# DredderGun/accbpg_and_fw

Hardware: AMD Instinct MI355X
Metric: D-opt iters/sec (m=2048,n=32768) (higher is better)
Workload: dtype f64; 1 GPU; D_opt_design(2048,32768) abpg_gain gamma=2 fp64, one independent instance per GPU; instances=1, instances_per_gpu=1, seeds=1..1, window=transient: iterations 5..161 from x0 = 1/n, linear_gram=False

## Files before the change

accbpg_and_fw_amd/csrc/dopt_kernels.hip:

```cpp
#include <atomic>
#include <mutex>
#include <unordered_map>
#include <type_traits>

#include "internal.h"
#include "mfma_tile.hpp"

namespace accbpg {

struct GramSeg {
    int64_t row0, col0, kb, ke;
    bool dual, whole;
};
constexpr int GRAM_RMAX = 4;
template <class T>
__device__ __forceinline__ GramSeg gram_segment(const TileRC* __restrict__ tiles, int64_t kiters, int64_t it,
                                                int64_t it1) {
    const int e = (int)(it / kiters);
    const int64_t off = it - (int64_t)e * kiters;
    const TileRC tr = tiles[e];
    GramSeg g;
    if (tr.d1 < 0) {
        g.row0 = (int64_t)tr.rb * T::BM; g.col0 = (int64_t)tr.cb * T::BN;
        g.kb = off; g.ke = min(kiters, off + (it1 - it));
// ... 1000 lines not shown
        const int c = 2 * (tid & 31), r0 = tid >> 5;
#pragma unroll
        for (int p = 0; p < 8; ++p) {
            const int r = r0 + 8 * p;
            v[p] = load2_guard(G + (int64_t)r * ld + c, r < mr, c, mc, vec_ok);
        }
    }
    __device__ __forceinline__ void to_lds(double* __restrict__ img, int st) const {
        const int tid = threadIdx.x;
        const int c = 2 * (tid & 31), r0 = tid >> 5;
#pragma unroll
        for (int p = 0; p < 8; ++p) {
            img[(r0 + 8 * p) * st + c] = v[p].x;
            img[(r0 + 8 * p) * st + c + 1] = v[p].y;
        }
    }
    __device__ __forceinline__ void from_lds(const double* __restrict__ img, int st) {
        const int tid = threadIdx.x;
        const int c = 2 * (tid & 31), r0 = tid >> 5;
#pragma unroll
        for (int p = 0; p < 8; ++p) {
            v[p].x = img[(r0 + 8 * p) * st + c];
            v[p].y = img[(r0 + 8 * p) * st + c + 1];
        }
    }
    __device__ __forceinline__ void store(double* __restrict__ G, int64_t ld, int mr, int mc, bool lower) const {
        const int tid = threadIdx.x;
        const int c = 2 * (tid & 31), r0 = tid >> 5;
#pragma unroll
        for (int p = 0; p < 8; ++p) {
            const int r = r0 + 8 * p;
            if (r < mr) {
                if (c < mc && (!lower || c <= r)) G[(int64_t)r * ld + c] = v[p].x;
                if (c + 1 < mc && (!lower || c + 1 <= r)) G[(int64_t)r * ld + c + 1] = v[p].y;
            }
        }
    }
};

__device__ __forceinline__ double rsqrt_newton(double d) {
    double y = __builtin_amdgcn_rsq(d);
    const double h = -0.5 * d;
    y = y * fma(h * y, y, 1.5);
    y = y * fma(h * y, y, 1.5);
    return y;
}

template <int SRC>
__device__ __forceinline__ double quad_bcast(double v) {
    constexpr int ctrl = SRC | (SRC << 2) | (SRC << 4) | (SRC << 6);
    int lo = __double2loint(v), hi = __double2hiint(v);
    lo = __builtin_amdgcn_mov_dpp(lo, ctrl, 0xF, 0xF, true);
    hi = __builtin_amdgcn_mov_dpp(hi, ctrl, 0xF, 0xF, true);
    return __hiloint2double(hi, lo);
}

__device__ __forceinline__ void solve16_quad(const double* P, double* X, int row, int k0,
                                             const double* __restrict__ lt, const double* __restrict__ rv) {
    const int q = threadIdx.x & 3;
    const double* prow = P + row * SP + k0;
    double* xr = X + row * SP + k0;
    double pr[4], xs[4];
#pragma unroll
    for (int t = 0; t < 4; ++t) pr[t] = prow[4 * t + q];
    double lv[2][4][4], rvv[2][4];
    auto group = [&](auto gtag) {
        constexpr int g = decltype(gtag)::value;
#pragma unroll
        for (int cc = 0; cc < 4; ++cc) {
            const int c = 4 * g + cc;
            rvv[g & 1][cc] = rv[c];
#pragma unroll
            for (int t = 0; t < 4; ++t)
                if (4 * t + 3 > c) lv[g & 1][cc][t] = lt[c * 16 + 4 * t + q];
        }
    };
    auto column = [&](auto ctag) {
        constexpr int c = decltype(ctag)::value;
        constexpr int qc = c & 3, tc = c >> 2, g = c >> 2;
        const double x = quad_bcast<qc>(pr[tc] * rvv[g & 1][c & 3]);
        xs[tc] = (q == qc) ? x : xs[tc];
#pragma unroll
        for (int t = 0; t < 4; ++t)
            if (4 * t + 3 > c) pr[t] = fma(-x, lv[g & 1][c & 3][t], pr[t]);
    };
    group(std::integral_constant<int, 0>{});
    group(std::integral_constant<int, 1>{});
    column(std::integral_constant<int, 0>{});  column(std::integral_constant<int, 1>{});
    column(std::integral_constant<int, 2>{});  column(std::integral_constant<int, 3>{});
    group(std::integral_constant<int, 2>{});
    column(std::integral_constant<int, 4>{});  column(std::integral_constant<int, 5>{});
    column(std::integral_constant<int, 6>{});  column(std::integral_constant<int, 7>{});
    group(std::integral_constant<int, 3>{});
    column(std::integral_constant<int, 8>{});  column(std::integral_constant<int, 9>{});
    column(std::integral_constant<int, 10>{}); column(std::integral_constant<int, 11>{});
    column(std::integral_constant<int, 12>{}); column(std::integral_constant<int, 13>{});
    column(std::integral_constant<int, 14>{}); column(std::integral_constant<int, 15>{});
#pragma unroll
    for (int t = 0; t < 4; ++t) xr[4 * t + q] = xs[t];
}

template <int SRC>
__device__ __forceinline__ double row_bcast(double v) {
    return __builtin_amdgcn_update_dpp(0.0, v, 0x150 + SRC, 0xF, 0xF, true);
}
#ifndef ACCBPG_DPP_ASM
#define ACCBPG_DPP_ASM 1
#endif
template <int C, int NOPS_BEFORE, int NOPS_AFTER>
__device__ __forceinline__ void fmac_row_bcast(double& acc, double l, double nl) {
#if ACCBPG_DPP_ASM
    if constexpr (NOPS_BEFORE) asm volatile("s_nop 1");
    asm volatile("v_fmac_f64_dpp %0, %1, %2 row_newbcast:%3 row_mask:0xf bank_mask:0xf"
                 : "+v"(acc)
                 : "v"(l), "v"(nl), "n"(C));
    if constexpr (NOPS_AFTER) asm volatile("s_nop 1");
#else
    acc = fma(row_bcast<C>(l), nl, acc);
#endif
}
template <int C>
__device__ __forceinline__ double mul_row_bcast(double y, double v) {
#if ACCBPG_DPP_ASM
    double out = 0.0;
    asm volatile("s_nop 1\n\tv_fmac_f64_dpp %0, %1, %2 row_newbcast:%3 row_mask:0xf bank_mask:0xf"
                 : "+v"(out)
                 : "v"(y), "v"(v), "n"(C));
    return out;
#else
    return fma(row_bcast<C>(y), v, 0.0);
#endif
}
template <int C0, int C1>
__device__ __forceinline__ void potrf16_updates(double (&a)[16], double l, double nl) {
    if constexpr (C0 < C1 && C0 < 16) {
        fmac_row_bcast<C0, 0, (C0 == 15)>(a[C0], l, nl);
        potrf16_updates<C0 + 1, C1>(a, l, nl);
    }
}
template <int J>
__device__ __forceinline__ void potrf16_step(double (&a)[16], double& l, int r, int k0, int bs, double& dsv,
                                             double& myrs, double& minp) {
    a[J] = l;
    if constexpr (J + 1 < 16) {
        const double nl = -l;
        fmac_row_bcast<J + 1, 1, 0>(a[J + 1], l, nl);
        const double p = a[J + 1];
        constexpr int N = 14 - J, Q = (N + 3) / 4;
        double y = __builtin_amdgcn_rsq(p);
        const double h = -0.5 * p;
        __builtin_amdgcn_sched_barrier(0);
        potrf16_updates<J + 2, J + 2 + Q>(a, l, nl);
        __builtin_amdgcn_sched_barrier(0);
        const double t = h * y;
        __builtin_amdgcn_sched_barrier(0);
        potrf16_updates<J + 2 + Q, J + 2 + 2 * Q>(a, l, nl);
        __builtin_amdgcn_sched_barrier(0);
        const double u = fma(t, y, 1.5);
        __builtin_amdgcn_sched_barrier(0);
        potrf16_updates<J + 2 + 2 * Q, J + 2 + 3 * Q>(a, l, nl);
        __builtin_amdgcn_sched_barrier(0);
        y = y * u;
        __builtin_amdgcn_sched_barrier(0);
        potrf16_updates<J + 2 + 3 * Q, 16>(a, l, nl);
        __builtin_amdgcn_sched_barrier(0);
        const bool mine = (r == J + 1);
        dsv = mine ? p : dsv;
        myrs = mine ? y : myrs;
        minp = (mine && (k0 + J + 1 < bs)) ? p : minp;
        l = mul_row_bcast<J + 1>(y, p);
    }
}
constexpr int POTRF_TB = 16 * 16 + 16;
struct PotrfNoHook { __device__ __forceinline__ void operator()(int, int) const {} };
template <class Hook = PotrfNoHook>
__device__ __forceinline__ void potrf64_blk(double* __restrict__ S, double* __restrict__ Lo,
                                            double* __restrict__ tbuf, int* __restrict__ badflag, int bs,
                                            int dbg = 0, Hook hook = Hook()) {
    const int tid = threadIdx.x;
    const int lane = tid & 63, wave = __builtin_amdgcn_readfirstlane(tid >> 6);
    for (int e = tid; e < 6 * 256; e += NTHREADS) {
        const int b = e >> 8, w = e & 255;
        const int br = (b < 3) ? 0 : ((b < 5) ? 1 : 2);
        const int bc = (b < 3) ? b + 1 : ((b < 5) ? b - 1 : 3);
        Lo[(16 * br + (w >> 4)) * SP + 16 * bc + (w & 15)] = 0.0;
    }
#pragma unroll 1
    for (int pnl = 0; pnl < NB / 16; ++pnl) {
        const int k0 = 16 * pnl;
        double* lt = tbuf + pnl * POTRF_TB;
        double* rv = lt + 256;
        if (wave == 0 && !(dbg & 32)) {
            const int r = lane & 15;
            double a[16];
#pragma unroll
            for (int c = 0; c < 16; ++c) a[c] = S[(k0 + r) * SP + k0 + c];
            double dsv = 1.0, myrs = 1.0, minp = 1.0;
            double l;
            {
                const double piv = row_bcast<0>(a[0]);
                const double rs = rsqrt_newton(piv);
                dsv = (r == 0) ? piv : dsv;
                myrs = (r == 0) ? rs : myrs;
                minp = (r == 0 && k0 < bs) ? piv : 1.0;
                l = a[0] * rs;
            }
            potrf16_step<0>(a, l, r, k0, bs, dsv, myrs, minp);
            potrf16_step<1>(a, l, r, k0, bs, dsv, myrs, minp);
            potrf16_step<2>(a, l, r, k0, bs, dsv, myrs, minp);
            potrf16_step<3>(a, l, r, k0, bs, dsv, myrs, minp);
            potrf16_step<4>(a, l, r, k0, bs, dsv, myrs, minp);
            potrf16_step<5>(a, l, r, k0, bs, dsv, myrs, minp);
            potrf16_step<6>(a, l, r, k0, bs, dsv, myrs, minp);
            potrf16_step<7>(a, l, r, k0, bs, dsv, myrs, minp);
            potrf16_step<8>(a, l, r, k0, bs, dsv, myrs, minp);
            potrf16_step<9>(a, l, r, k0, bs, dsv, myrs, minp);
            potrf16_step<10>(a, l, r, k0, bs, dsv, myrs, minp);
            potrf16_step<11>(a, l, r, k0, bs, dsv, myrs, minp);
            potrf16_step<12>(a, l, r, k0, bs, dsv, myrs, minp);
            potrf16_step<13>(a, l, r, k0, bs, dsv, myrs, minp);
            potrf16_step<14>(a, l, r, k0, bs, dsv, myrs, minp);
            potrf16_step<15>(a, l, r, k0, bs, dsv, myrs, minp);
            const bool bad = __any(!(minp > 0.0));
            const double dg = sqrt(dsv);
            if (lane < 16) {
#pragma unroll
                for (int c = 0; c < 16; ++c) {
                    const double v = (c < r) ? a[c] : ((c == r) ? dg : 0.0);
                    Lo[(k0 + r) * SP + k0 + c] = v;
                    lt[c * 16 + r] = v;
                }
                rv[r] = myrs;
                if (bad) *badflag = 1;
            }
        } else {
            hook(pnl, 3);
        }
        hook(pnl, 0);
        __syncthreads();
        hook(pnl, 1);
        if (pnl == NB / 16 - 1) break;
        const int nrows = NB - k0 - 16;
        if (tid < 4 * nrows && !(dbg & 8)) {
            const int row = k0 + 16 + (tid >> 2);
            solve16_quad(S, Lo, row, k0, lt, rv);
        }
        __syncthreads();
        {
            const int nb = NB / 16 - 1 - pnl;
            const int nblk = nb * (nb + 1) / 2;
            const int lr = lane & 15, lq = lane >> 4;
            for (int b = wave; b < nblk && !(dbg & 16); b += NTHREADS / 64) {
                int bi = 0;
                while ((bi + 1) * (bi + 2) / 2 <= b) ++bi;
                const int bj = b - bi * (bi + 1) / 2;
                const int ri = 16 * (pnl + 1 + bi), rj = 16 * (pnl + 1 + bj);
                d4 acc = d4{0.0, 0.0, 0.0, 0.0};
#pragma unroll
                for (int kk = 0; kk < 4; ++kk) {
                    const double av = Lo[(ri + lr) * SP + k0 + 4 * kk + lq];
                    const double bv = Lo[(rj + lr) * SP + k0 + 4 * kk + lq];
                    acc = __builtin_amdgcn_mfma_f64_16x16x4f64(av, bv, acc, 0, 0, 0);
                }
#pragma unroll
                for (int rr = 0; rr < 4; ++rr) S[(ri + lq + 4 * rr) * SP + rj + lr] -= acc[rr];
            }
        }
        __syncthreads();
    }
}

__device__ __forceinline__ void trsm64_blk(double* __restrict__ Xs, const double* __restrict__ Lo,
                                           const double* __restrict__ tbuf) {
    const int tid = threadIdx.x;
    const int lane = tid & 63, wave = __builtin_amdgcn_readfirstlane(tid >> 6);
#pragma unroll 1
    for (int pnl = 0; pnl < NB / 16; ++pnl) {
        const int k0 = 16 * pnl;
        const double* lt = tbuf + pnl * POTRF_TB;
        const double* rv = lt + 256;
        solve16_quad(Xs, Xs, tid >> 2, k0, lt, rv);
        if (pnl == NB / 16 - 1) break;
        __syncthreads();
        {
            const int ncb = NB / 16 - 1 - pnl;
            const int lr = lane & 15, lq = lane >> 4;
            for (int b = wave; b < 4 * ncb; b += NTHREADS / 64) {
                const int bi = b & 3, q = pnl + 1 + (b >> 2);
                d4 acc = d4{0.0, 0.0, 0.0, 0.0};
#pragma unroll
                for (int kk = 0; kk < 4; ++kk) {
                    const double av = Xs[(16 * bi + lr) * SP + k0 + 4 * kk + lq];
                    const double bv = Lo[(16 * q + lr) * SP + k0 + 4 * kk + lq];
                    acc = __builtin_amdgcn_mfma_f64_16x16x4f64(av, bv, acc, 0, 0, 0);
                }
#pragma unroll
                for (int rr = 0; rr < 4; ++rr) Xs[(16 * bi + lq + 4 * rr) * SP + 16 * q + lr] -= acc[rr];
            }
        }
        __syncthreads();
    }
}

template <class Fetch, class Done>
__device__ __forceinline__ bool trsm64_stream(double* __restrict__ Xs, const double* __restrict__ Lo,
                                              const double* __restrict__ tbuf, Fetch fetch, Done done) {
    const int tid = threadIdx.x;
    const int lane = tid & 63, wave = __builtin_amdgcn_readfirstlane(tid >> 6);
#pragma unroll 1
    for (int pnl = 0; pnl < NB / 16; ++pnl) {
        const int k0 = 16 * pnl;
        const double* lt = tbuf + pnl * POTRF_TB;
        const double* rv = lt + 256;
        if (!fetch(pnl, 0)) return false;
        if (pnl + 1 < NB / 16) fetch(pnl + 1, 1);
        solve16_quad(Xs, Xs, tid >> 2, k0, lt, rv);
        if (pnl + 1 < NB / 16) fetch(pnl + 1, 2);
        __syncthreads();
        if (!done(pnl)) return false;
        if (pnl == NB / 16 - 1) break;
        {
            const int ncb = NB / 16 - 1 - pnl;
            const int lr = lane & 15, lq = lane >> 4;
            for (int b = wave; b < 4 * ncb; b += NTHREADS / 64) {
                const int bi = b & 3, q = pnl + 1 + (b >> 2);
                d4 acc = d4{0.0, 0.0, 0.0, 0.0};
#pragma unroll
                for (int kk = 0; kk < 4; ++kk) {
                    const double av = Xs[(16 * bi + lr) * SP + k0 + 4 * kk + lq];
                    const double bv = Lo[(16 * q + lr) * SP + k0 + 4 * kk + lq];
                    acc = __builtin_amdgcn_mfma_f64_16x16x4f64(av, bv, acc, 0, 0, 0);
                }
#pragma unroll
                for (int rr = 0; rr < 4; ++rr) Xs[(16 * bi + lq + 4 * rr) * SP + 16 * q + lr] -= acc[rr];
            }
        }
    }
    return true;
}

__global__ __launch_bounds__(NTHREADS, 1) void chol_step_kernel(double* __restrict__ A, int64_t lda, int64_t m,
                                                               int kc, int pend, int jmax, int T,
                                                               double* __restrict__ logdet,
                                                               int* __restrict__ flags, int dbg,
                                                               double* __restrict__ Winv, double* __restrict__ Ldiag) {
    extern __shared__ __attribute__((aligned(16))) double lds[];
    double* Ak = lds;
    double* Bk = Ak + NB * SQ;
    double* S = Bk + NB * SQ;
    double* Lo = S + NB * SP;
    double* misc = Lo + NB * SP;
    int* badflag = reinterpret_cast<int*>(misc);
    double* red = misc + 8;
    const int tid = threadIdx.x;
    const int kprev = pend ? kc - 1 : -1;
    const int npanel = T - kc;
    const bool vec_ok = ((reinterpret_cast<uintptr_t>(A) & 15) == 0) && ((lda & 1) == 0);
    const double* Lk = A + (int64_t)(kc - 1) * NB;
    acc64_t acc;

    if ((int)blockIdx.x >= npanel) {
        const int u = blockIdx.x - npanel;
        int ii, jj;
        if (jmax >= T - 1) {
            ii = (int)((sqrt(8.0 * u + 1.0) - 1.0) * 0.5);
            while ((ii + 1) * (ii + 2) / 2 <= u) ++ii;
            while (ii * (ii + 1) / 2 > u) --ii;
            jj = u - ii * (ii + 1) / 2;
        } else {
            const int J = jmax - kc;
            ii = u / J; jj = u - ii * J;
            if (jj > ii) return;
        }
        const int i = kc + 1 + ii, j = kc + 1 + jj;
        const int mi = (int)min((int64_t)NB, m - (int64_t)i * NB), mj = (int)min((int64_t)NB, m - (int64_t)j * NB);
        Blk64 bi, bj, bc;
        bi.load(Lk + (int64_t)i * NB * lda, lda, mi, NB, vec_ok);
        bj.load(Lk + (int64_t)j * NB * lda, lda, mj, NB, vec_ok);
        double* Cij = A + (int64_t)i * NB * lda + (int64_t)j * NB;
        bc.load(Cij, lda, mi, mj, vec_ok);
        bi.to_lds(Ak, SQ);
        bj.to_lds(Bk, SQ);
        bc.to_lds(S, SP);
        __syncthreads();
        mma64(acc, Ak, Bk);
        sub_acc64(S, acc, mi, mj, i == j);
        __syncthreads();
        bc.from_lds(S, SP);
        bc.store(Cij, lda, mi, mj, i == j);
        return;
    }

    const int i = kc + blockIdx.x;
    const bool diag = (i == kc);
    const int bs = (int)min((int64_t)NB, m - (int64_t)kc * NB);
    const int mi = (int)min((int64_t)NB, m - (int64_t)i * NB);
    double* Akk = A + (int64_t)kc * NB * lda + (int64_t)kc * NB;
    double* Pik = A + (int64_t)i * NB * lda + (int64_t)kc * NB;
    Blk64 bkk, bik, bd, bp;
    bd.load(Akk, lda, bs, bs, vec_ok);
    if (kprev >= 0) bkk.load(Lk + (int64_t)kc * NB * lda, lda, bs, NB, vec_ok);
    if (!diag) {
        bp.load(Pik, lda, mi, bs, vec_ok);
        if (kprev >= 0) bik.load(Lk + (int64_t)i * NB * lda, lda, mi, NB, vec_ok);
    }
    {
        const int c = 2 * (tid & 31), r0 = tid >> 5;
#pragma unroll
        for (int p = 0; p < 8; ++p) {
            const int r = r0 + 8 * p;
            const bool in = r < bs;
            S[r * SP + c] = (in && c <= r) ? bd.v[p].x : ((r == c) ? 1.0 : 0.0);
            S[r * SP + c + 1] = (in && c + 1 <= r && c + 1 < bs) ? bd.v[p].y : ((r == c + 1) ? 1.0 : 0.0);
        }
    }
    if (tid == 0) *badflag = 0;
    acc64_t pacc;
    if (kprev >= 0) {
        bkk.to_lds(Bk, SQ);
        if (!diag) bik.to_lds(Ak, SQ);
        __syncthreads();
        if (!(dbg & 4)) {
            mma64(acc, Bk, Bk);
            if (!diag) mma64(pacc, Ak, Bk);
            sub_acc64(S, acc, bs, bs, true);
        }
    }
    __syncthreads();
    if (!(dbg & 1)) potrf64_blk(S, Lo, Ak, badflag, bs, dbg);
    else { __syncthreads(); for (int e = tid; e < NB * SP; e += NTHREADS) Lo[e] = S[e]; __syncthreads(); }
    const bool bad = (*badflag != 0);
    if (diag) {
        Blk64 bl;
        bl.from_lds(Lo, SP);
        bl.store(Ldiag + (int64_t)kc * NB * lda + (int64_t)kc * NB, lda, bs, bs, true);
        double lg = (tid < bs) ? log(Lo[tid * SP + tid]) : 0.0;
        for (int off = 32; off > 0; off >>= 1) lg += __shfl_down(lg, off);
        if ((tid & 63) == 0) red[tid >> 6] = lg;
        __syncthreads();
        if (tid == 0) {
#if defined(ACCBPG_PLAIN_LOGDET) && ACCBPG_PLAIN_LOGDET
            *logdet += 2.0 * (red[0] + red[1] + red[2] + red[3]);
#else
            __hip_atomic_fetch_add(logdet, 2.0 * (red[0] + red[1] + red[2] + red[3]), __ATOMIC_RELAXED,
                                   __HIP_MEMORY_SCOPE_AGENT);
#endif
            if (bad) flags[FLAG_NOT_PD] = 1;
        }
        if (Winv != nullptr) {
            __syncthreads();
            for (int e = tid; e < NB * NB; e += NTHREADS) S[(e >> 6) * SP + (e & 63)] = ((e >> 6) == (e & 63)) ? 1.0 : 0.0;
            __syncthreads();
            trsm64_blk(S, Lo, Ak);
            __syncthreads();
            double* Wkk = Winv + (int64_t)kc * NB * lda + (int64_t)kc * NB;
            for (int e = tid; e < NB * NB; e += NTHREADS) {
                const int r = e >> 6, c = e & 63;
                if (r < bs && c < bs) Wkk[(int64_t)r * lda + c] = (c <= r) ? S[c * SP + r] : 0.0;
            }
        }
        return;
    }
    double* Xs = S;
    bp.to_lds(Xs, SP);
    __syncthreads();
    if (kprev >= 0 && !(dbg & 4)) sub_acc64(Xs, pacc, mi, bs, false);
    __syncthreads();
    if (!(dbg & 2)) trsm64_blk(Xs, Lo, Ak);
    __syncthreads();
    bp.from_lds(Xs, SP);
    bp.store(Pik, lda, mi, bs, false);
}

__device__ __forceinline__ void mma64_acc(acc64_t& acc, const double* __restrict__ As, const double* __restrict__ Bs) {
    const int lane = threadIdx.x & 63, wave = __builtin_amdgcn_readfirstlane(threadIdx.x >> 6);
    const int wm = wave >> 1, wn = wave & 1;
    const int lr = lane & 15, lq = lane >> 4;
    const double* ap = As + (16 * wm + lr) * SQ + lq;
    const double* bp = Bs + (32 * wn + lr) * SQ + lq;
#pragma unroll 4
    for (int kk = 0; kk < NB / 4; ++kk) {
        const double a0 = ap[4 * kk], a1 = ap[32 * SQ + 4 * kk];
        const double b0 = bp[4 * kk], b1 = bp[16 * SQ + 4 * kk];
        acc[0][0] = __builtin_amdgcn_mfma_f64_16x16x4f64(a0, b0, acc[0][0], 0, 0, 0);
        acc[0][1] = __builtin_amdgcn_mfma_f64_16x16x4f64(a0, b1, acc[0][1], 0, 0, 0);
        acc[1][0] = __builtin_amdgcn_mfma_f64_16x16x4f64(a1, b0, acc[1][0], 0, 0, 0);
        acc[1][1] = __builtin_amdgcn_mfma_f64_16x16x4f64(a1, b1, acc[1][1], 0, 0, 0);
    }
}

__global__ __launch_bounds__(NTHREADS, 2) void chol_syrk_kernel(double* __restrict__ A, int64_t lda, int64_t m,
                                                               int k0, int nk, int T) {
    extern __shared__ __attribute__((aligned(16))) double lds[];
    double* Ak = lds;
    double* Bk = Ak + NB * SQ;
    double* S = Ak;
    const bool vec_ok = ((reinterpret_cast<uintptr_t>(A) & 15) == 0) && ((lda & 1) == 0);
    const int u = blockIdx.x;
    int ii = (int)((sqrt(8.0 * u + 1.0) - 1.0) * 0.5);
    while ((ii + 1) * (ii + 2) / 2 <= u) ++ii;
    while (ii * (ii + 1) / 2 > u) --ii;
    const int jj = u - ii * (ii + 1) / 2;
    const int i = k0 + nk + ii, j = k0 + nk + jj;
    if (i >= T) return;
    const int mi = (int)min((int64_t)NB, m - (int64_t)i * NB), mj = (int)min((int64_t)NB, m - (int64_t)j * NB);
    double* Cij = A + (int64_t)i * NB * lda + (int64_t)j * NB;
    const double* Li = A + (int64_t)i * NB * lda + (int64_t)k0 * NB;
    const double* Lj = A + (int64_t)j * NB * lda + (int64_t)k0 * NB;
    Blk64 bi, bj, bc;
    bc.load(Cij, lda, mi, mj, vec_ok);
    bi.load(Li, lda, mi, NB, vec_ok);
    bj.load(Lj, lda, mj, NB, vec_ok);
    acc64_t acc;
#pragma unroll
    for (int a = 0; a < 2; ++a)
#pragma unroll
        for (int b = 0; b < 2; ++b) acc[a][b] = d4{0.0, 0.0, 0.0, 0.0};
#pragma unroll 1
    for (int k = 0; k < nk; ++k) {
        bi.to_lds(Ak, SQ);
        bj.to_lds(Bk, SQ);
        if (k + 1 < nk) {
            bi.load(Li + (int64_t)(k + 1) * NB, lda, mi, NB, vec_ok);
            bj.load(Lj + (int64_t)(k + 1) * NB, lda, mj, NB, vec_ok);
        }
        __syncthreads();
        mma64_acc(acc, Ak, Bk);
        __syncthreads();
    }
    bc.to_lds(S, SP);
    __syncthreads();
    sub_acc64(S, acc, mi, mj, i == j);
    __syncthreads();
    bc.from_lds(S, SP);
    bc.store(Cij, lda, mi, mj, i == j);
}

constexpr int CT_TMAX = 32;
constexpr int CT_AUX = 4 * POTRF_TB + 8;
constexpr int CT_LDS_DOUBLES = 2 * NB * SQ + 4 * POTRF_TB + 16;
constexpr int CT_LDS_BYTES = CT_LDS_DOUBLES * 8;

constexpr int CT_NSTAMP = 32;

typedef __attribute__((address_space(1))) double gdouble;
typedef __attribute__((address_space(1))) int gint;
__device__ __forceinline__ double ct_ld(const double* p) {
    return __hip_atomic_load((const gdouble*)p, __ATOMIC_RELAXED, __HIP_MEMORY_SCOPE_AGENT);
}
__device__ __forceinline__ void ct_st(double* p, double v) {
    __hip_atomic_store((gdouble*)p, v, __ATOMIC_RELAXED, __HIP_MEMORY_SCOPE_AGENT);
}
__device__ __forceinline__ int ct_ldi(const int* p) {
    return __hip_atomic_load((const gint*)p, __ATOMIC_RELAXED, __HIP_MEMORY_SCOPE_AGENT);
}
__device__ __forceinline__ void ct_sti(int* p, int v) {
    __hip_atomic_store((gint*)p, v, __ATOMIC_RELAXED, __HIP_MEMORY_SCOPE_AGENT);
}
__device__ __forceinline__ bool ct_spin(const int* flag, int* abortw, long long limit) {
    if (ct_ldi(flag) != 0) return true;
    const long long t0 = wall_clock64();
    unsigned n = 0;
    for (;;) {
        __builtin_amdgcn_s_sleep(1);
        if (ct_ldi(flag) != 0) return true;
        if ((++n & 15u) == 0u) {
            if (ct_ldi(abortw) != 0) return false;
            if (wall_clock64() - t0 > limit) {
                ct_sti(abortw, 1);
                return false;
            }
        }
    }
}
__device__ __forceinline__ bool ct_wait(const int* f0, const int* f1, int* abortw, long long limit, int* word) {
    if (threadIdx.x < 64) {
        bool ok = ct_spin(f0, abortw, limit);
        if (ok && f1 != nullptr) ok = ct_spin(f1, abortw, limit);
        if (threadIdx.x == 0) *word = ok ? 1 : 0;
    }
    __syncthreads();
    return *word != 0;
}
template <int ST, bool LOWER>
__device__ __forceinline__ void ct_fetch(double* __restrict__ img, const double* G, int64_t ld, int mr, int mc) {
    const int tid = threadIdx.x;
    const int c = 2 * (tid & 31), r0 = tid >> 5;
    double v[16];
#pragma unroll
    for (int p = 0; p < 8; ++p) {
        const int r = r0 + 8 * p;
        const bool in0 = r < mr && c < mc && (!LOWER || c <= r);
        const bool in1 = r < mr && c + 1 < mc && (!LOWER || c + 1 <= r);
        v[2 * p] = in0 ? ct_ld(G + (int64_t)r * ld + c) : 0.0;
        v[2 * p + 1] = in1 ? ct_ld(G + (int64_t)r * ld + c + 1) : 0.0;
    }
#pragma unroll
    for (int p = 0; p < 8; ++p) {
        img[(r0 + 8 * p) * ST + c] = v[2 * p];
        img[(r0 + 8 * p) * ST + c + 1] = v[2 * p + 1];
    }
}
template <bool LOWER>
__device__ __forceinline__ void ct_publish(const double* __restrict__ img, double* G, int64_t ld, int mr, int mc) {
    const int tid = threadIdx.x;
    const int c = 2 * (tid & 31), r0 = tid >> 5;
#pragma unroll
    for (int p = 0; p < 8; ++p) {
        const int r = r0 + 8 * p;
        if (r < mr) {
            if (c < mc && (!LOWER || c <= r)) ct_st(G + (int64_t)r * ld + c, img[r * SP + c]);
            if (c + 1 < mc && (!LOWER || c + 1 <= r)) ct_st(G + (int64_t)r * ld + c + 1, img[r * SP + c + 1]);
        }
    }
}
__device__ __forceinline__ void ct_signal(int* flag) {
    asm volatile("s_waitcnt vmcnt(0)" ::: "memory");
    __syncthreads();
    if (threadIdx.x == 0) ct_sti(flag, 1);
}
__device__ __forceinline__ void ct_load_acc(acc64_t& acc, const double* __restrict__ G, int64_t ld, int mr, int mc) {
    const int lane = threadIdx.x & 63, wave = __builtin_amdgcn_readfirstlane(threadIdx.x >> 6);
    const int wm = wave >> 1, wn = wave & 1;
    const int lr = lane & 15, lq = lane >> 4;
#pragma unroll
    for (int i = 0; i < 2; ++i)
#pragma unroll
        for (int j = 0; j < 2; ++j)
#pragma unroll
            for (int r = 0; r < 4; ++r) {
                const int row = 16 * (2 * i + wm) + lq + 4 * r, col = 32 * wn + 16 * j + lr;
                acc[i][j][r] = (row < mr && col < mc) ? G[(int64_t)row * ld + col] : 0.0;
            }
}
template <bool DIAG>
__device__ __forceinline__ void ct_acc_to_img(double* __restrict__ img, const acc64_t& acc, int bs) {
    const int lane = threadIdx.x & 63, wave = __builtin_amdgcn_readfirstlane(threadIdx.x >> 6);
    const int wm = wave >> 1, wn = wave & 1;
    const int lr = lane & 15, lq = lane >> 4;
#pragma unroll
    for (int i = 0; i < 2; ++i)
#pragma unroll
        for (int j = 0; j < 2; ++j)
#pragma unroll
            for (int r = 0; r < 4; ++r) {
                const int row = 16 * (2 * i + wm) + lq + 4 * r, col = 32 * wn + 16 * j + lr;
                double v = acc[i][j][r];
                if (DIAG) v = (row < bs && col < bs && col <= row) ? v : ((row == col) ? 1.0 : 0.0);
                img[row * SP + col] = v;
            }
}
template <int SA, int SB>
__device__ __forceinline__ void ct_update(acc64_t& acc, const double* __restrict__ As, const double* __restrict__ Bs) {
    const int lane = threadIdx.x & 63, wave = __builtin_amdgcn_readfirstlane(threadIdx.x >> 6);
    const int wm = wave >> 1, wn = wave & 1;
    const int lr = lane & 15, lq = lane >> 4;
    const double* ap = As + (16 * wm + lr) * SA + lq;
    const double* bp = Bs + (32 * wn + lr) * SB + lq;
    d4 p00 = d4{0.0, 0.0, 0.0, 0.0}, p01 = p00, p10 = p00, p11 = p00;
#pragma unroll 4
    for (int kk = 0; kk < NB / 4; ++kk) {
        const double a0 = ap[4 * kk], a1 = ap[32 * SA + 4 * kk];
        const double b0 = bp[4 * kk], b1 = bp[16 * SB + 4 * kk];
        p00 = __builtin_amdgcn_mfma_f64_16x16x4f64(a0, b0, p00, 0, 0, 0);
        p01 = __builtin_amdgcn_mfma_f64_16x16x4f64(a0, b1, p01, 0, 0, 0);
        p10 = __builtin_amdgcn_mfma_f64_16x16x4f64(a1, b0, p10, 0, 0, 0);
        p11 = __builtin_amdgcn_mfma_f64_16x16x4f64(a1, b1, p11, 0, 0, 0);
    }
    acc[0][0] -= p00; acc[0][1] -= p01; acc[1][0] -= p10; acc[1][1] -= p11;
}

__global__ __launch_bounds__(NTHREADS, 2) void chol_tiles_kernel(CholInst one, const CholInst* __restrict__ table,
                                                                const CholJob* __restrict__ jobs, int64_t ld, int64_t m,
                                                                int T, long long spin_limit, int stall_test, BatchAct act) {
    extern __shared__ __attribute__((aligned(16))) double lds[];
    double* R0 = lds;
    double* R1 = R0 + NB * SQ;
    double* tbuf = R1 + NB * SQ;
    int* word = reinterpret_cast<int*>(tbuf + 4 * POTRF_TB);
    int* badflag = word + 2;
    double* red = tbuf + 4 * POTRF_TB + 8;

    const CholInst ci = (table != nullptr) ? table[act.idx[blockIdx.y]] : one;
    const CholJob job = jobs[blockIdx.x];
    const int tid = threadIdx.x;
    const bool diagrole = (job.i == job.j);
    const int d = job.i;
    const bool has_off = !diagrole || d > 0;
    const int ti = job.i, tj = diagrole ? d - 1 : job.j;
    int* abortw = ci.flags + FLAG_ABORT;
    int* pflags = ci.ready + T * T;
    int* hflags = pflags + 4 * T;
    auto blk = [&](int b) { return (int)min((int64_t)NB, m - (int64_t)b * NB); };
    auto at = [&](auto* base, int bi, int bj) { return base + (int64_t)bi * NB * ld + (int64_t)bj * NB; };
    if (stall_test && blockIdx.x == 0) return;
    auto stamp = [&](int slot) {
        if (ci.trace != nullptr && diagrole && tid == 0) ci.trace[d * CT_NSTAMP + slot] = wall_clock64();
    };
    stamp(0);

    acc64_t accO, accD;
    const int mi = blk(ti);
    if (has_off) ct_load_acc(accO, at(ci.src, ti, tj), ld, mi, blk(tj));
    if (diagrole && d < 2) ct_load_acc(accD, at(ci.src, d, d), ld, blk(d), blk(d));

    double run_logdet = 0.0, run_bad = 0.0;
    if (has_off) {
        for (int k = 0; k < tj; ++k) {
            if (!ct_wait(ci.ready + ti * T + k, nullptr, abortw, spin_limit, word)) return;
            ct_fetch<SQ, false>(R0, at(ci.L, ti, k), ld, mi, NB);
            if (!ct_wait(ci.ready + tj * T + k, nullptr, abortw, spin_limit, word)) return;
            ct_fetch<SQ, false>(R1, at(ci.L, tj, k), ld, blk(tj), NB);
            __syncthreads();
            ct_update<SQ, SQ>(accO, R0, R1);
        }
        __syncthreads();
        ct_acc_to_img<false>(R0, accO, NB);
        stamp(1);
        const double* ax = ci.aux + (int64_t)tj * CT_AUX;
        const double* Ljj = at(ci.Ldiag, tj, tj);
        int* pflag = pflags + 4 * tj;
        double pc_t[2], pc_l[3], pc_s[2];
        bool have = false;
        int looked = 0;
        auto load_piece = [&](int pnl) {
            const int k0 = 16 * pnl;
#pragma unroll
            for (int q = 0; q < 2; ++q) {
                const int e = tid + q * NTHREADS;
                pc_t[q] = (e < POTRF_TB) ? ct_ld(ax + pnl * POTRF_TB + e) : 0.0;
            }
#pragma unroll
            for (int q = 0; q < 3; ++q) {
                const int e = tid + q * NTHREADS;
                pc_l[q] = (e < (NB - k0 - 16) * 16) ? ct_ld(Ljj + (int64_t)(k0 + 16 + (e >> 4)) * ld + k0 + (e & 15)) : 0.0;
            }
            if (pnl == 3) {
                pc_s[0] = ct_ld(ax + 4 * POTRF_TB);
                pc_s[1] = ct_ld(ax + 4 * POTRF_TB + 1);
            }
        };
        auto land_piece = [&](int pnl) {
            const int k0 = 16 * pnl;
#pragma unroll
            for (int q = 0; q < 2; ++q) {
                const int e = tid + q * NTHREADS;
                if (e < POTRF_TB) tbuf[pnl * POTRF_TB + e] = pc_t[q];
            }
#pragma unroll
            for (int q = 0; q < 3; ++q) {
                const int e = tid + q * NTHREADS;
                if (e < (NB - k0 - 16) * 16) R1[(k0 + 16 + (e >> 4)) * SP + k0 + (e & 15)] = pc_l[q];
            }
            if (pnl == 3) { run_logdet = pc_s[0]; run_bad = pc_s[1]; }
        };
        auto fetch = [&](int pnl, int mode) -> bool {
            if (mode == 1) { looked = ct_ldi(pflag + pnl); return true; }
            if (mode == 2) { if (looked != 0) { load_piece(pnl); have = true; } return true; }
            stamp(8 + 4 * pnl + (have ? 0 : 0));
            if (have) land_piece(pnl);
            if (__syncthreads_or(have ? 0 : 1)) {
                if (!ct_wait(pflag + pnl, nullptr, abortw, spin_limit, word)) return false;
                if (!have) { load_piece(pnl); land_piece(pnl); }
                __syncthreads();
            }
            have = false;
            stamp(9 + 4 * pnl);
            if (pnl == 0) stamp(2);
            if (pnl == 3) stamp(3);
            return true;
        };
        double* Lij = at(ci.L, ti, tj);
        const int mj = blk(tj);
        d4 p00 = d4{0.0, 0.0, 0.0, 0.0}, p01 = p00, p10 = p00, p11 = p00;
        auto done = [&](int pnl) -> bool {
            const int k0 = 16 * pnl;
            stamp(10 + 4 * pnl);
            for (int e = tid; e < NB * 16; e += NTHREADS) {
                const int r = e >> 4, c = k0 + (e & 15);
                if (r < mi && c < mj) ct_st(Lij + (int64_t)r * ld + c, R0[r * SP + c]);
            }
            if (diagrole) {
                const int lane = tid & 63, wave = __builtin_amdgcn_readfirstlane(tid >> 6);
                const int wm = wave >> 1, wn = wave & 1;
                const double* ap = R0 + (16 * wm + (lane & 15)) * SP + (lane >> 4);
                const double* bp = R0 + (32 * wn + (lane & 15)) * SP + (lane >> 4);
#pragma unroll
                for (int kk = 4 * pnl; kk < 4 * pnl + 4; ++kk) {
                    const double a0 = ap[4 * kk], a1 = ap[32 * SP + 4 * kk];
                    const double b0 = bp[4 * kk], b1 = bp[16 * SP + 4 * kk];
                    p00 = __builtin_amdgcn_mfma_f64_16x16x4f64(a0, b0, p00, 0, 0, 0);
                    p01 = __builtin_amdgcn_mfma_f64_16x16x4f64(a0, b1, p01, 0, 0, 0);
                    p10 = __builtin_amdgcn_mfma_f64_16x16x4f64(a1, b0, p10, 0, 0, 0);
                    p11 = __builtin_amdgcn_mfma_f64_16x16x4f64(a1, b1, p11, 0, 0, 0);
                }
                if (pnl == 2 && d >= 2) {
                    if (!ct_wait(hflags + d, nullptr, abortw, spin_limit, word)) return false;
                    const double* hd = ci.hand + (int64_t)d * NB * NB;
#pragma unroll
                    for (int i = 0; i < 2; ++i)
#pragma unroll
                        for (int j = 0; j < 2; ++j)
#pragma unroll
                            for (int r = 0; r < 4; ++r) accD[i][j][r] = ct_ld(hd + ((i * 2 + j) * 4 + r) * NTHREADS + tid);
                }
            }
            stamp(11 + 4 * pnl);
            if (pnl == 3) stamp(4);
            return true;
        };
        if (!trsm64_stream(R0, R1, tbuf, fetch, done)) return;
        if (!diagrole) {
            ct_signal(ci.ready + ti * T + tj);
            if (tj != 0) return;
            acc64_t accH;
            ct_load_acc(accH, at(ci.src, ti, ti), ld, mi, mi);
            for (int k = 0; k + 1 < ti; ++k) {
                if (!ct_wait(ci.ready + ti * T + k, nullptr, abortw, spin_limit, word)) return;
                ct_fetch<SQ, false>(R0, at(ci.L, ti, k), ld, mi, NB);
                __syncthreads();
                ct_update<SQ, SQ>(accH, R0, R0);
            }
            double* hd = ci.hand + (int64_t)ti * NB * NB;
#pragma unroll
            for (int i = 0; i < 2; ++i)
#pragma unroll
                for (int j = 0; j < 2; ++j)
#pragma unroll
                    for (int r = 0; r < 4; ++r) ct_st(hd + ((i * 2 + j) * 4 + r) * NTHREADS + tid, accH[i][j][r]);
            ct_signal(hflags + ti);
            return;
        }
        accD[0][0] -= p00; accD[0][1] -= p01; accD[1][0] -= p10; accD[1][1] -= p11;
    }
    const int bs = blk(d);
    ct_acc_to_img<true>(R1, accD, bs);
    if (tid == 0) *badflag = 0;
    asm volatile("s_waitcnt vmcnt(0)" ::: "memory");
    __syncthreads();
    if (has_off && tid == 0) ct_sti(ci.ready + ti * T + tj, 1);
    stamp(5);
    double* axd = ci.aux + (int64_t)d * CT_AUX;
    double* Ldd = at(ci.Ldiag, d, d);
    int* pflag_d = pflags + 4 * d;
    auto publish_piece = [&](int pnl, int first, int nthr) {
        const int k0 = 16 * pnl;
        for (int e = tid - first; e < (NB - k0) * 16; e += nthr) {
            const int r = k0 + (e >> 4), c = k0 + (e & 15);
            if (r < bs && c <= r) ct_st(Ldd + (int64_t)r * ld + c, R0[r * SP + c]);
        }
        for (int e = tid - first; e < POTRF_TB; e += nthr) ct_st(axd + pnl * POTRF_TB + e, tbuf[pnl * POTRF_TB + e]);
    };
    auto hook = [&](int pnl, int where) {
        if (where == 3 && pnl > 0) publish_piece(pnl - 1, 64, NTHREADS - 64);
        else if (where == 0 && pnl > 0) asm volatile("s_waitcnt vmcnt(0)" ::: "memory");
        else if (where == 1 && pnl > 0 && tid == 0) ct_sti(pflag_d + pnl - 1, 1);
    };
    potrf64_blk(R1, R0, tbuf, badflag, bs, 0, hook);
    stamp(6);
    double lg = (tid < bs) ? log(R0[tid * SP + tid]) : 0.0;
    for (int off = 32; off > 0; off >>= 1) lg += __shfl_down(lg, off);
    if ((tid & 63) == 0) red[tid >> 6] = lg;
    publish_piece(3, 0, NTHREADS);
    __syncthreads();
    const double logdet = run_logdet + 2.0 * (red[0] + red[1] + red[2] + red[3]);
    const double bad = (*badflag != 0 || run_bad != 0.0) ? 1.0 : 0.0;
    if (tid == 0) { ct_st(axd + 4 * POTRF_TB, logdet); ct_st(axd + 4 * POTRF_TB + 1, bad); }
    ct_signal(pflag_d + 3);
    stamp(7);
    if (d == T - 1 && tid == 0) {
        *ci.logdet = logdet;
        if (bad != 0.0) ci.flags[FLAG_NOT_PD] = 1;
    }
    if (ci.Winv != nullptr) {
        for (int e = tid; e < NB * NB; e += NTHREADS) R1[(e >> 6) * SP + (e & 63)] = ((e >> 6) == (e & 63)) ? 1.0 : 0.0;
        __syncthreads();
        trsm64_blk(R1, R0, tbuf);
        __syncthreads();
        double* Wkk = at(ci.Winv, d, d);
        for (int e = tid; e < NB * NB; e += NTHREADS) {
            const int r = e >> 6, c = e & 63;
            if (r < bs && c < bs) Wkk[(int64_t)r * ld + c] = (c <= r) ? R1[c * SP + r] : 0.0;
        }
    }
}

__global__ __launch_bounds__(64) void trtri_diag_kernel(const double* __restrict__ L, int64_t ldl,
                                                       double* __restrict__ W, int64_t ldw, int64_t m) {
    __shared__ double Ls[NB * SP];
    __shared__ double Ws[NB * SP];
    __shared__ double rinv[NB];
    const int tid = threadIdx.x;
    const int64_t k0 = (int64_t)blockIdx.x * NB;
    const int bs = (int)min((int64_t)NB, m - k0);
    const double* L11 = L + k0 * ldl + k0;
    for (int e = tid; e < NB * NB; e += 64) {
        const int r = e / NB, c = e % NB;
        Ls[r * SP + c] = (r < bs && c <= r) ? L11[(int64_t)r * ldl + c] : ((r == c) ? 1.0 : 0.0);
    }
    __syncthreads();
    rinv[tid] = 1.0 / Ls[tid * SP + tid];
    __syncthreads();
    double w[NB];
#pragma unroll
    for (int r = 0; r < NB; ++r) {
        double s = (r == tid) ? 1.0 : 0.0;
#pragma unroll
        for (int c = 0; c < r; ++c) s -= Ls[r * SP + c] * w[c];
        w[r] = (r >= tid) ? s * rinv[r] : 0.0;
    }
#pragma unroll
    for (int r = 0; r < NB; ++r) Ws[r * SP + tid] = w[r];
    __syncthreads();
    double* W11 = W + k0 * ldw + k0;
    for (int e = tid; e < NB * NB; e += 64) {
        const int r = e / NB, c = e % NB;
        if (r < bs && c < bs) W11[(int64_t)r * ldw + c] = Ws[r * SP + c];
    }
}

template <bool COPY = false>
__device__ __forceinline__ bool xcheck_bad(const double* __restrict__ x, int64_t n, double* __restrict__ keep = nullptr) {
    bool bad = false;
    const int64_t step = (int64_t)blockDim.x * 8;
    int64_t i = threadIdx.x;
    for (; i + 7 * (int64_t)blockDim.x < n; i += step) {
        double v[8];
#pragma unroll
        for (int u = 0; u < 8; ++u) v[u] = x[i + u * (int64_t)blockDim.x];
#pragma unroll
        for (int u = 0; u < 8; ++u) {
            bad |= !(v[u] >= 0.0);
            if (COPY) keep[i + u * (int64_t)blockDim.x] = v[u];
        }
    }
    for (; i < n; i += blockDim.x) {
        const double v = x[i];
        bad |= !(v >= 0.0);
        if (COPY) keep[i] = v;
    }
    return __syncthreads_or(bad ? 1 : 0) != 0;
}

__global__ __launch_bounds__(1024) void zero_scalars_kernel(double* dscal, int* dflag, const double* __restrict__ x,
                                                          int64_t n, int* __restrict__ ready, int nready,
                                                          double* __restrict__ xkeep) {
#if defined(ACCBPG_PLAIN_LOGDET) && ACCBPG_PLAIN_LOGDET
    if (threadIdx.x < 8) dscal[threadIdx.x] = 0.0;
#else
    if (threadIdx.x < 8) __hip_atomic_store(dscal + threadIdx.x, 0.0, __ATOMIC_RELAXED, __HIP_MEMORY_SCOPE_AGENT);
#endif
    if (threadIdx.x < 8) dflag[threadIdx.x] = 0;
    for (int i = threadIdx.x; i < nready; i += blockDim.x) ready[i] = 0;
    if (x == nullptr) return;
    const bool bad = xkeep ? xcheck_bad<true>(x, n, xkeep) : xcheck_bad<false>(x, n);
    if (bad && threadIdx.x == 0) dflag[FLAG_NEG_X] = 1;
}

__global__ __launch_bounds__(1024) void zero_scalars_batch_kernel(const BatchInst* __restrict__ bt, BatchAct act,
                                                                const double* __restrict__ xbase, int64_t ldx, int64_t n,
                                                                int nready) {
    const int inst = act.idx[blockIdx.x];
    const BatchInst bi = bt[inst];
    if (threadIdx.x < 8) __hip_atomic_store(bi.dscal + threadIdx.x, 0.0, __ATOMIC_RELAXED, __HIP_MEMORY_SCOPE_AGENT);
    if (threadIdx.x < 8) bi.dflag[threadIdx.x] = 0;
    for (int i = threadIdx.x; i < nready; i += blockDim.x) bi.chol_ready[i] = 0;
    if (xbase == nullptr) return;
    if (xcheck_bad(xbase + (int64_t)inst * ldx, n) && threadIdx.x == 0) bi.dflag[FLAG_NEG_X] = 1;
}

__global__ void set_op_kernel(GemmOp* slot, GemmOp op) { *slot = op; }

__global__ __launch_bounds__(NTHREADS, 1) void mfma_peak_kernel(int iters, double* sink) {
    d4 acc[8];
#pragma unroll
    for (int i = 0; i < 8; ++i) acc[i] = d4{0.0, 0.0, 0.0, 0.0};
    double a = 1.0 + threadIdx.x * 1e-3, b = 0.5 - threadIdx.x * 1e-3;
    for (int it = 0; it < iters; ++it) {
#pragma unroll
        for (int i = 0; i < 8; ++i)
            asm volatile("v_mfma_f64_16x16x4_f64 %0, %1, %2, %0" : "+v"(acc[i]) : "v"(a), "v"(b));
    }
    asm volatile("s_nop 15\n\ts_nop 15" ::: "memory");
    double s = 0.0;
#pragma unroll
    for (int i = 0; i < 8; ++i) s += acc[i][0] + acc[i][1] + acc[i][2] + acc[i][3];
    if (s == 123.456) sink[0] = s;
}

__global__ __launch_bounds__(NTHREADS, 1) void pipe_probe_kernel(int iters, int mode, double* sink) {
    d4 acc[8];
    double va[16];
#pragma unroll
    for (int i = 0; i < 8; ++i) acc[i] = d4{0.0, 0.0, 0.0, 0.0};
#pragma unroll
    for (int i = 0; i < 16; ++i) va[i] = threadIdx.x * 1e-3 + i;
    double a = 1.0 + threadIdx.x * 1e-3, b = 0.5 - threadIdx.x * 1e-3;
    for (int it = 0; it < iters; ++it) {
        if (mode & 1) {
#pragma unroll
            for (int i = 0; i < 8; ++i) asm volatile("v_mfma_f64_16x16x4_f64 %0, %1, %2, %0" : "+v"(acc[i]) : "v"(a), "v"(b));
        }
        if (mode & 2) {
#pragma unroll
            for (int r = 0; r < 8; ++r)
#pragma unroll
                for (int i = 0; i < 16; ++i) asm volatile("v_fma_f64 %0, %1, %2, %0" : "+v"(va[i]) : "v"(a), "v"(b));
        }
    }
    asm volatile("s_nop 15\n\ts_nop 15" ::: "memory");
    double s = 0.0;
#pragma unroll
    for (int i = 0; i < 8; ++i) s += acc[i][0] + acc[i][1] + acc[i][2] + acc[i][3];
#pragma unroll
    for (int i = 0; i < 16; ++i) s += va[i];
    if (s == 123.456) sink[0] = s;
}

template <class K>
static int set_lds(K kernel, int bytes) {
    ACC_HIP(hipFuncSetAttribute(reinterpret_cast<const void*>(kernel), hipFuncAttributeMaxDynamicSharedMemorySize,
                                bytes));
    return ACCBPG_OK;
}

static int ensure_lds(const void* kernel, int bytes) {
    static std::mutex mu;
    static std::unordered_map<const void*, int> limit;
    std::lock_guard<std::mutex> guard(mu);
    auto it = limit.find(kernel);
    if (it != limit.end() && it->second >= bytes) return ACCBPG_OK;
    ACC_HIP(hipFuncSetAttribute(kernel, hipFuncAttributeMaxDynamicSharedMemorySize, bytes));
    limit[kernel] = bytes;
    return ACCBPG_OK;
}
#define ACC_LAUNCH_LDS(kernel, grid, block, lds, stream, ...)                        \
    do {                                                                             \
        auto k__ = kernel;                                                           \
        ACC_TRY(ensure_lds(reinterpret_cast<const void*>(k__), (int)(lds)));         \
        k__<<<(grid), (block), (lds), (stream)>>>(__VA_ARGS__);                      \
    } while (0)

void prof_begin(accbpg_dopt* h, ProfKind k) {
    if (!h->prof_on) return;
    ProfSlot& p = h->prof[k];
    if (p.used + 2 > p.ev.size()) {
        hipEvent_t a, b;
        hipEventCreate(&a);
        hipEventCreate(&b);
        p.ev.push_back(a);
        p.ev.push_back(b);
    }
    hipEventRecord(p.ev[p.used], h->stream);
}
void prof_end(accbpg_dopt* h, ProfKind k) {
    if (!h->prof_on) return;
    ProfSlot& p = h->prof[k];
    hipEventRecord(p.ev[p.used + 1], h->stream);
    p.used += 2;
    p.launches += 1;
}

static int g_plan_flags = 0;
void set_plan_flags(int flags) { g_plan_flags = flags; }

static std::atomic<int> g_gemm_loop{0};
int set_gemm_loop(int variant) {
    if (variant < 0 || variant > 4) return ACCBPG_ERR_ARG;
    g_gemm_loop.store(variant);
    return ACCBPG_OK;
}
template <int LOOP>
static int set_lds_gemm_loop() {
    ACC_TRY(set_lds(gemm_ops_kernel<TileSmall<true>, LOOP>, TileSmall<true>::LDS_BYTES));
    ACC_TRY(set_lds(gemm_ops_kernel<TileSmall<false>, LOOP>, TileSmall<false>::LDS_BYTES));
    return ACCBPG_OK;
}
static int set_lds_gemm_ops() {
    ACC_TRY(set_lds_gemm_loop<0>());
    ACC_TRY(set_lds_gemm_loop<2>());
    ACC_TRY(set_lds_gemm_loop<3>());
    ACC_TRY(set_lds_gemm_loop<4>());
    return ACCBPG_OK;
}
template <class F>
static int with_gemm_loop(F&& f) {
    switch (g_gemm_loop.load()) {
        case 0: return f(std::integral_constant<int, GEMM_LOOP_DEPTH>{});
        case 1: return f(std::integral_constant<int, 0>{});
        case 2: return f(std::integral_constant<int, 2>{});
        case 3: return f(std::integral_constant<int, 3>{});
        default: return f(std::integral_constant<int, 4>{});
    }
}

int build_plans(accbpg_dopt* h) {
    const int64_t m = h->m;
    const bool interior256 = h->vec_ok && (m % 256 == 0) && (h->n % BK == 0);
    const int BM = h->big ? TileBig<false>::BM : TileSmall<false>::BM;
    const int BN = h->big ? TileBig<false>::BN : TileSmall<false>::BN;
    std::vector<TileRC> tl;
    const int nrb = (int)((m + BM - 1) / BM), ncb = (int)((m + BN - 1) / BN);
    h->gram_chunks = 1;
    h->gram_nc = h->n;
    constexpr int64_t GRAM_NC = 32768;
    if (!(g_plan_flags & 4) && h->big && interior256 && h->use_glds && h->n >= 2 * GRAM_NC && h->n % GRAM_NC == 0) {
        h->gram_chunks = (int)(h->n / GRAM_NC);
// ... 828 lines not shown
```

Baseline: 65.18 iterations/s.

## Unroll streamed TRSM panels, prefetch diagonal hand-off and next panel earlier

Replaces the generic strided right-update loop in the streamed 64-wide TRSM with a per-wave templated update that keeps operands in registers and fully unrolls the panel loop. It adds an extra prefetch point after each panel's right-update. The diagonal hand-off accumulator load, previously a blocking wait inside panel 2, is now polled and prefetched early, with a blocking wait only as a fallback at panel 3. The intent is to hide flag waits and global-load latency behind MFMA work, at the cost of more registers, more code, and a custom LDS-based vote that replaces __syncthreads_or.

```diff
diff --git a/accbpg_and_fw_amd/csrc/dopt_kernels.hip b/accbpg_and_fw_amd/csrc/dopt_kernels.hip
--- a/accbpg_and_fw_amd/csrc/dopt_kernels.hip
+++ b/accbpg_and_fw_amd/csrc/dopt_kernels.hip
@@ -1326,12 +1326,45 @@
     }
 }
 
+template <int NCB>
+__device__ __forceinline__ void trsm_right_update(double* __restrict__ Xs, const double* __restrict__ Lo, int pnl,
+                                                  int wave, int lane) {
+    static_assert(NTHREADS / 64 == 4, "one 16-row block of the tile per wave");
+    const int k0 = 16 * pnl;
+    const int lr = lane & 15, lq = lane >> 4;
+    const double* ap = Xs + (16 * wave + lr) * SP + k0 + lq;
+    const double* bp = Lo + (16 * (pnl + 1) + lr) * SP + k0 + lq;
+    double* cp = Xs + (16 * wave + lq) * SP + 16 * (pnl + 1) + lr;
+    double av[4], bv[NCB][4], cv[NCB][4];
+#pragma unroll
+    for (int kk = 0; kk < 4; ++kk) av[kk] = ap[4 * kk];
+#pragma unroll
+    for (int j = 0; j < NCB; ++j)
+#pragma unroll
+        for (int kk = 0; kk < 4; ++kk) bv[j][kk] = bp[16 * j * SP + 4 * kk];
+#pragma unroll
+    for (int j = 0; j < NCB; ++j)
+#pragma unroll
+        for (int rr = 0; rr < 4; ++rr) cv[j][rr] = cp[4 * rr * SP + 16 * j];
+    d4 acc[NCB];
+#pragma unroll
+    for (int j = 0; j < NCB; ++j) acc[j] = d4{0.0, 0.0, 0.0, 0.0};
+#pragma unroll
+    for (int kk = 0; kk < 4; ++kk)
+#pragma unroll
+        for (int j = 0; j < NCB; ++j) acc[j] = __builtin_amdgcn_mfma_f64_16x16x4f64(av[kk], bv[j][kk], acc[j], 0, 0, 0);
+#pragma unroll
+    for (int j = 0; j < NCB; ++j)
+#pragma unroll
+        for (int rr = 0; rr < 4; ++rr) cp[4 * rr * SP + 16 * j] = cv[j][rr] - acc[j][rr];
+}
+
 template <class Fetch, class Done>
 __device__ __forceinline__ bool trsm64_stream(double* __restrict__ Xs, const double* __restrict__ Lo,
                                               const double* __restrict__ tbuf, Fetch fetch, Done done) {
     const int tid = threadIdx.x;
     const int lane = tid & 63, wave = __builtin_amdgcn_readfirstlane(tid >> 6);
-#pragma unroll 1
+#pragma unroll
     for (int pnl = 0; pnl < NB / 16; ++pnl) {
         const int k0 = 16 * pnl;
         const double* lt = tbuf + pnl * POTRF_TB;
@@ -1343,22 +1376,10 @@
         __syncthreads();
         if (!done(pnl)) return false;
         if (pnl == NB / 16 - 1) break;
-        {
-            const int ncb = NB / 16 - 1 - pnl;
-            const int lr = lane & 15, lq = lane >> 4;
-            for (int b = wave; b < 4 * ncb; b += NTHREADS / 64) {
-                const int bi = b & 3, q = pnl + 1 + (b >> 2);
-                d4 acc = d4{0.0, 0.0, 0.0, 0.0};
-#pragma unroll
-                for (int kk = 0; kk < 4; ++kk) {
-                    const double av = Xs[(16 * bi + lr) * SP + k0 + 4 * kk + lq];
-                    const double bv = Lo[(16 * q + lr) * SP + k0 + 4 * kk + lq];
-                    acc = __builtin_amdgcn_mfma_f64_16x16x4f64(av, bv, acc, 0, 0, 0);
-                }
-#pragma unroll
-                for (int rr = 0; rr < 4; ++rr) Xs[(16 * bi + lq + 4 * rr) * SP + 16 * q + lr] -= acc[rr];
-            }
-        }
+        if (pnl + 1 < NB / 16) fetch(pnl + 1, 3);
+        if (pnl == 0) trsm_right_update<3>(Xs, Lo, pnl, wave, lane);
+        else if (pnl == 1) trsm_right_update<2>(Xs, Lo, pnl, wave, lane);
+        else trsm_right_update<1>(Xs, Lo, pnl, wave, lane);
     }
     return true;
 }
@@ -1719,7 +1740,8 @@
     auto at = [&](auto* base, int bi, int bj) { return base + (int64_t)bi * NB * ld + (int64_t)bj * NB; };
     if (stall_test && blockIdx.x == 0) return;
     auto stamp = [&](int slot) {
-        if (ci.trace != nullptr && diagrole && tid == 0) ci.trace[d * CT_NSTAMP + slot] = wall_clock64();
+        if (ci.trace != nullptr && diagrole && tid == 0)
+            ((__attribute__((address_space(1))) long long*)ci.trace)[d * CT_NSTAMP + slot] = wall_clock64();
     };
     stamp(0);
 
@@ -1747,6 +1769,18 @@
         double pc_t[2], pc_l[3], pc_s[2];
         bool have = false;
         int looked = 0;
+        const bool wantD = diagrole && d >= 2;
+        bool haveD = false;
+        int lookedD = 0;
+        auto load_diag = [&]() {
+            const double* hd = ci.hand + (int64_t)d * NB * NB;
+#pragma unroll
+            for (int i = 0; i < 2; ++i)
+#pragma unroll
+                for (int j = 0; j < 2; ++j)
+#pragma unroll
+                    for (int r = 0; r < 4; ++r) accD[i][j][r] = ct_ld(hd + ((i * 2 + j) * 4 + r) * NTHREADS + tid);
+        };
         auto load_piece = [&](int pnl) {
             const int k0 = 16 * pnl;
 #pragma unroll
@@ -1778,14 +1812,67 @@
             }
             if (pnl == 3) { run_logdet = pc_s[0]; run_bad = pc_s[1]; }
         };
+        auto land_now = [&](int pnl) {
+            const int k0 = 16 * pnl;
+            double t_t[2], t_l[3];
+#pragma unroll
+            for (int q = 0; q < 2; ++q) {
+                const int e = tid + q * NTHREADS;
+                t_t[q] = (e < POTRF_TB) ? ct_ld(ax + pnl * POTRF_TB + e) : 0.0;
+            }
+#pragma unroll
+            for (int q = 0; q < 3; ++q) {
+                const int e = tid + q * NTHREADS;
+                t_l[q] = (e < (NB - k0 - 16) * 16) ? ct_ld(Ljj + (int64_t)(k0 + 16 + (e >> 4)) * ld + k0 + (e & 15)) : 0.0;
+            }
+            if (pnl == 3) {
+                run_logdet = ct_ld(ax + 4 * POTRF_TB);
+                run_bad = ct_ld(ax + 4 * POTRF_TB + 1);
+            }
+#pragma unroll
+            for (int q = 0; q < 2; ++q) {
+                const int e = tid + q * NTHREADS;
+                if (e < POTRF_TB) tbuf[pnl * POTRF_TB + e] = t_t[q];
+            }
+#pragma unroll
+            for (int q = 0; q < 3; ++q) {
+                const int e = tid + q * NTHREADS;
+                if (e < (NB - k0 - 16) * 16) R1[(k0 + 16 + (e >> 4)) * SP + k0 + (e & 15)] = t_l[q];
+            }
+        };
+        auto vote_any = [&](bool mine) -> bool {
+            int* votes = word + 4;
+            const int any = __any(mine ? 1 : 0);
+            if ((tid & 63) == 0) votes[tid >> 6] = any;
+            __syncthreads();
+            return (votes[0] | votes[1] | votes[2] | votes[3]) != 0;
+        };
         auto fetch = [&](int pnl, int mode) -> bool {
-            if (mode == 1) { looked = ct_ldi(pflag + pnl); return true; }
-            if (mode == 2) { if (looked != 0) { load_piece(pnl); have = true; } return true; }
+            if (mode == 1) {
+                looked = ct_ldi(pflag + pnl);
+                if (wantD && !haveD) lookedD = ct_ldi(hflags + d);
+                return true;
+            }
+            if (mode == 3) {
+                if (!have && looked != 0) { load_piece(pnl); have = true; }
+                return true;
+            }
+            if (mode == 2) {
+                if (looked != 0) { load_piece(pnl); have = true; }
+                else looked = ct_ldi(pflag + pnl);
+                if (wantD && !haveD && lookedD != 0) { load_diag(); haveD = true; }
+                return true;
+            }
             stamp(8 + 4 * pnl + (have ? 0 : 0));
             if (have) land_piece(pnl);
-            if (__syncthreads_or(have ? 0 : 1)) {
+            const bool needD = pnl == 3 && wantD;
+            if (vote_any(!(have && (!needD || haveD)))) {
+                if (needD) {
+                    if (!ct_wait(hflags + d, nullptr, abortw, spin_limit, word)) return false;
+                    if (!haveD) { load_diag(); haveD = true; }
+                }
                 if (!ct_wait(pflag + pnl, nullptr, abortw, spin_limit, word)) return false;
-                if (!have) { load_piece(pnl); land_piece(pnl); }
+                if (!have) land_now(pnl);
                 __syncthreads();
             }
             have = false;
@@ -1817,16 +1904,6 @@
                     p01 = __builtin_amdgcn_mfma_f64_16x16x4f64(a0, b1, p01, 0, 0, 0);
                     p10 = __builtin_amdgcn_mfma_f64_16x16x4f64(a1, b0, p10, 0, 0, 0);
                     p11 = __builtin_amdgcn_mfma_f64_16x16x4f64(a1, b1, p11, 0, 0, 0);
-                }
-                if (pnl == 2 && d >= 2) {
-                    if (!ct_wait(hflags + d, nullptr, abortw, spin_limit, word)) return false;
-                    const double* hd = ci.hand + (int64_t)d * NB * NB;
-#pragma unroll
-                    for (int i = 0; i < 2; ++i)
-#pragma unroll
-                        for (int j = 0; j < 2; ++j)
-#pragma unroll
-                            for (int r = 0; r < 4; ++r) accD[i][j][r] = ct_ld(hd + ((i * 2 + j) * 4 + r) * NTHREADS + tid);
                 }
             }
             stamp(11 + 4 * pnl);
```

New measurement: 66.05 iterations/s, median of 6. +1.3%, better.
